# hadleyhzy34/porl

Measured on AMD Instinct MI355X. Metric: gradient-steps/sec (POR update, batch=1024), higher is better.
Workload: dtype f32; 1 GPU; POR S=60 A=2 H=1024 L=2 B=1024/GPU (global 1024), 1000000 -row replay (1000000/GPU) resident in HBM, device sampler + gather + full update per step; parallelism=dp1, global_batch=1024

## Files before the change

### porl_amd/csrc/iql_api.inc

```

namespace {

int64_t add_tensor(std::vector<TensorInfo>& v, int64_t& cur, int rows, int cols) {
  const int64_t off = cur;
  v.push_back({off, rows, cols});
  cur += ru4((int64_t)(rows ? rows : 1) * cols);
  return off;
}

void layout_mlp(MlpLayout& m, std::vector<TensorInfo>& v, int64_t& cur, int in, int hid, int L, int out, bool ln) {
  m.n_lin = L + 1;
  m.ln = ln;
  m.dims[0] = in;
  for (int l = 0; l < L; ++l) m.dims[l + 1] = hid;
  m.dims[L + 1] = out;
  for (int l = 0; l <= L; ++l) {
    m.w[l] = add_tensor(v, cur, m.dims[l + 1], m.dims[l]);
    m.b[l] = add_tensor(v, cur, 0, m.dims[l + 1]);
    if (ln && l < L) {
      m.lnw[l] = add_tensor(v, cur, 0, hid);
      m.lnb[l] = add_tensor(v, cur, 0, hid);
    }
  }
}

struct Workspace {
  int64_t xs_slot[PORL_IQL_SLOTS], xt_slot[PORL_IQL_SLOTS], target_v_slot[PORL_IQL_SLOTS];
  int64_t xn, rew, term;
  int64_t act_v[2][PORL_MAX_HIDDEN], act_t[2][2], act_p[PORL_MAX_HIDDEN];
  int64_t dz_v[2][2], dz_p[2];
  int64_t hp_t[2], hp_v[2];
  int64_t act_q[2][2], hp_q[2];
  int64_t dv[2], dmu;
  int64_t slab_mean, slab_a, slab_b, slab_pa;
  int64_t part_loss, part_min, part_dls;
  int64_t xhat_v[2][PORL_MAX_HIDDEN], rstd_v[2][PORL_MAX_HIDDEN];
  int64_t ln_dg[2], ln_db[2], ln_dh[2];
  int64_t head_part[2], head_loss, head_db[2];
  int64_t pol_w;
  int64_t total;
};

}

struct porl_iql {
  porl_iql_cfg cfg;
  MlpLayout v[2], pol;
  int64_t logstd_off = 0, n_vf = 0, n_pol = 0;
  std::vector<TensorInfo> t_vf, t_pol;
  porl_iql_buffers buf{};
  bool bound = false;
  int device = -1;
  int mode = 0;
  int slot = 0;
  ReduceArgs fin_v{}, fin_p{};
  bool fin_v_pending = false, fin_p_pending = false;
  int batch = 0;
  bool have_pol_target = false;
  bool pol_prefetched = false;
  bool pol_fwd_done = false;
  int pol_nslab = 1;
  int Sp = 0, Dp = 0, Hp = 0, parts_max = 0;
  Workspace ws{};
  Tune tune = g_tune;
};

namespace {

int check_ready(const porl_iql* h, bool need_batch) {
  if (!h) PORL_FAIL(PORL_ERR_INVALID, "null engine");
  if (!h->bound) PORL_FAIL(PORL_ERR_UNBOUND, "porl_iql_bind() has not been called");
  if (need_batch && h->batch <= 0) PORL_FAIL(PORL_ERR_INVALID, "no minibatch loaded (porl_iql_load_batch)");
  return 0;
}
int iql_enter(const porl_iql* h, bool need_batch, const porl_iql_hyper* hp) {
  PORL_TRY(check_ready(h, need_batch));
  if (!hp) PORL_FAIL(PORL_ERR_INVALID, "null hyper-parameters");
  return 0;
// ... 184 lines not shown
  for (int i = 0; i < nnets; ++i) if (!skn_ok4(nets[i].dz, ldz)) return false;
  WgradSkinnyArgs a{};
  a.nnets = nnets; a.B = B; a.H = H; a.S = S; a.ldz = ldz; a.ldx = ldx; a.ldo = S;
  a.tiles_n = cdiv(H, SKN_T);
  skn_split(cdiv(B, SKN_T), h->tune.dw0_slabs, a.nslab, a.rtiles);
  a.slabW_stride = (long)H * S; a.slabC_stride = H;
  for (int i = 0; i < nnets; ++i) {
    a.net[i] = WgradSkinnyNet{nets[i].dz, X, nets[i].sl.W, nets[i].sl.C};
    add_reduce(red, nets[i].gw, nets[i].sl.W, (long)H * S, (long)H * S, a.nslab);
    add_reduce(red, nets[i].gb, nets[i].sl.C, H, H, a.nslab);
  }
  g_phase = phase;
  {
    ProfScope ps("wgrad_skinny_kernel", s, 2.0 * nnets * B * (double)H * S,
                 4.0 * nnets * ((double)B * H + (double)B * S + (double)a.nslab * H * (S + 1)));
    hipLaunchKernelGGL(wgrad_skinny_kernel, dim3(nnets * a.nslab * a.tiles_n), dim3(256), 0, s, a);
  }
  g_phase = "";
  const hipError_t e = hipGetLastError();
  if (e != hipSuccess) { g_err = std::string("wgrad_skinny_kernel: ") + hipGetErrorString(e); *rc = (int)e; }
  return true;
}

int combine_or_defer(ReduceArgs& red, ReduceArgs* defer, hipStream_t s) {
  if (defer) { *defer = red; return 0; }
  return launch_reduce(red, s);
}

int value_forward(porl_iql* h, hipStream_t s, int* parts) {
  const int S = h->cfg.obs_dim, H = h->cfg.hidden_dim, L = h->cfg.n_hidden;
  const Workspace& ws = h->ws;
  for (int l = 0; l < L; ++l) {
    FwdNet nets[4];
    for (int i = 0; i < 2; ++i) {
      nets[i] = twin_fwd_net(h, h->buf.params_tgt, i, l, ws.xn, ws.act_t[i], false, ws.hp_t[i]);
      nets[2 + i] = twin_fwd_net(h, h->buf.params_vf, i, l, ws.xs_slot[h->slot], ws.act_v[i], true, ws.hp_v[i]);
    }
    g_phase = l == 0 ? "V2.L0fwd:" : "V3.fwd:";
    PORL_TRY(fwd_hidden_layer(h, nets, 4, h->batch, l == 0 ? S : H, l == L - 1, parts, false, s));
  }
  g_phase = "V4.head:";
  return PORL_OK;
}

int value_backward_ln(porl_iql* h, const porl_iql_hyper* hp, hipStream_t s, int parts, ReduceArgs* defer) {
  const int B = h->batch, S = h->cfg.obs_dim, H = h->cfg.hidden_dim, L = h->cfg.n_hidden, Hp = h->Hp;
  float* W = h->buf.workspace;
  const Workspace& ws = h->ws;
  const float* Pv = h->buf.params_vf;
  const float* Pt = h->buf.params_tgt;
  float* Gv = h->buf.grads_vf;
  {
    ValueLossArgs a{};
    for (int i = 0; i < 2; ++i) {
      a.hp_t[i] = W + ws.hp_t[i]; a.hp_v[i] = W + ws.hp_v[i];
      a.b_t[i] = Pt + h->v[i].b[L]; a.b_v[i] = Pv + h->v[i].b[L];
      a.dv[i] = W + ws.dv[i];
      a.db_out[i] = Gv + h->v[i].b[L];
    }
    a.rew = W + ws.rew; a.term = W + ws.term; a.target_v = W + ws.target_v_slot[h->slot]; a.stats = h->buf.stats;
    a.B = B; a.parts = parts; a.tau = hp->tau; a.discount = hp->discount; a.inv_batch = hp->inv_batch;
    hipLaunchKernelGGL(value_loss_kernel, dim3(1), dim3(1024), 0, s, a);
    PORL_HIP(hipGetLastError());
  }
  const int nln = cdiv(B, LN_ROWS_PER_BLOCK);
  for (int l = L - 1; l >= 0; --l) {
    const bool top = l == L - 1;
    {
// ... 15 lines not shown
        add_reduce(r, Gv + h->v[i].lnw[l], W + ws.ln_dg[i], H, H, nln);
        add_reduce(r, Gv + h->v[i].lnb[l], W + ws.ln_db[i], H, H, nln);
        if (top) add_reduce(r, Gv + h->v[i].w[L], W + ws.ln_dh[i], H, H, nln);
      }
      PORL_TRY(launch_reduce(r, s));
    }
    ReduceArgs red{};
    GemmGroup g{};
    for (int i = 0; i < 2; ++i) {
      const MlpLayout& m = h->v[i];
      BwdNet n{W + ws.dz_v[i][1], nullptr, Hp, Gv + m.w[l], Gv + m.b[l], Pv + m.w[l], nullptr, nullptr};
      if (l == 0) { n.in = W + ws.xs_slot[h->slot]; n.ldin = h->Sp; }
      else { n.in = W + ws.act_v[i][l - 1]; n.dz_prev = W + ws.dz_v[i][0]; }
      bwd_layer_group(h, g, n, l == 0 ? S : H);
    }
    const int tile = iql_tile(h, g);
    if (l == 0) dw0_splitk(h, g, tile, 2, SLAB_TWIN0, red);
    PORL_TRY(iql_launch(h, g, tile, false, s));
    PORL_TRY(combine_or_defer(red, l == 0 ? defer : nullptr, s));
  }
  return PORL_OK;
}

int value_backward_relu(porl_iql* h, const porl_iql_hyper* hp, hipStream_t s, int parts, ReduceArgs* defer) {
  const int B = h->batch, S = h->cfg.obs_dim, H = h->cfg.hidden_dim, L = h->cfg.n_hidden, Hp = h->Hp;
  float* W = h->buf.workspace;
  const Workspace& ws = h->ws;
  const float* Pv = h->buf.params_vf;
  const float* Pt = h->buf.params_tgt;
  float* Gv = h->buf.grads_vf;
  ReduceArgs red{};
  {
    const int nhb = cdiv(B, HEAD_ROWS_PER_BLOCK);
    HeadBwdArgs a{};
    for (int i = 0; i < 2; ++i) {
      a.Hact[i] = W + ws.act_v[i][L - 1]; a.w[i] = Pv + h->v[i].w[L];
      a.dZ[i] = W + ws.dz_v[i][(L - 1) & 1]; a.part_dw[i] = W + ws.head_part[i];
      a.hp_t[i] = W + ws.hp_t[i]; a.hp_v[i] = W + ws.hp_v[i];
      a.b_t[i] = Pt + h->v[i].b[L]; a.b_v[i] = Pv + h->v[i].b[L];
      a.dv[i] = W + ws.dv[i]; a.part_db[i] = W + ws.head_db[i];
      add_reduce(red, Gv + h->v[i].w[L], W + ws.head_part[i], H, H, nhb);
      add_reduce(red, Gv + h->v[i].b[L], W + ws.head_db[i], 1, 1, nhb);
    }
    a.rew = W + ws.rew; a.term = W + ws.term; a.target_v = W + ws.target_v_slot[h->slot]; a.part_loss = W + ws.head_loss;
    add_reduce(red, h->buf.stats, W + ws.head_loss, 1, 1, nhb, 0, hp->inv_batch);
    a.B = B; a.H = H; a.ld = Hp; a.parts = parts;
    a.tau = hp->tau; a.discount = hp->discount; a.inv_batch = hp->inv_batch;
    ProfScope ps("relu_head_bwd_kernel", s, 0.0, 16.0 * B * H);
    hipLaunchKernelGGL(relu_head_bwd_kernel, dim3(nhb, 2), dim3(256), 0, s, a);
    PORL_HIP(hipGetLastError());
  }
  for (int l = L - 1; l >= 0; --l) {
    if (l == 0) {
      Dw0Net dn[2];
      for (int i = 0; i < 2; ++i) dn[i] = Dw0Net{W + ws.dz_v[i][0], Gv + h->v[i].w[0], Gv + h->v[i].b[0], slabs(h, SlabSet(SLAB_TWIN0 + i))};
      int rc = 0;
      if (dw0_skinny(h, dn, 2, red, "V6.dW0:", s, &rc)) {
        if (rc) return rc;
        break;
      }
    }
    GemmGroup g{};
    for (int i = 0; i < 2; ++i) {
      const MlpLayout& m = h->v[i];
      BwdNet n{W + ws.dz_v[i][l & 1], nullptr, Hp, Gv + m.w[l], Gv + m.b[l], Pv + m.w[l], nullptr, nullptr};
      if (l == 0) { n.in = W + ws.xs_slot[h->slot]; n.ldin = h->Sp; }
      else { n.in = n.mask = W + ws.act_v[i][l - 1]; n.dz_prev = W + ws.dz_v[i][(l - 1) & 1]; }
      bwd_layer_group(h, g, n, l == 0 ? S : H);
    }
    int tile = iql_tile(h, g);
    if (l > 0 && short_blocks(h) && h->tune.vbwd_tile_short >= 0) tile = h->tune.vbwd_tile_short;
    if (l == 0) dw0_splitk(h, g, tile, 2, SLAB_TWIN0, red);
    g_phase = l == 0 ? "V6.dW0:" : "V5.bwd:";
    PORL_TRY(iql_launch(h, g, tile, false, s));
  }
  g_phase = "V7.combine:";
  PORL_TRY(combine_or_defer(red, defer, s));
  g_phase = "";
  return PORL_OK;
}

int value_backward_impl(porl_iql* h, const porl_iql_hyper* hp, hipStream_t s, ReduceArgs* defer) {
  int parts = 0;
  PORL_TRY(value_forward(h, s, &parts));
  return h->cfg.layer_norm ? value_backward_ln(h, hp, s, parts, defer) : value_backward_relu(h, hp, s, parts, defer);
}

int value_adam(porl_iql* h, const porl_iql_hyper* hp, hipStream_t s, const ReduceArgs* fin) {
  g_phase = "V8.";
  const int rc = adam_launch(h->buf.params_vf, h->buf.grads_vf, h->buf.adam_m_vf, h->buf.adam_v_vf, h->buf.params_tgt, h->n_vf,
                             hp->value_lr, hp->value_step, hp->adam_beta1, hp->adam_beta2, hp->adam_eps, hp->ema_beta, s, fin);
  g_phase = "";
  return rc;
}

int policy_adam(porl_iql* h, const porl_iql_hyper* hp, hipStream_t s, const ReduceArgs* fin, const char* phase) {
  g_phase = phase;
  const int rc = adam_launch(h->buf.params_pol, h->buf.grads_pol, h->buf.adam_m_pol, h->buf.adam_v_pol, nullptr, h->n_pol,
                             hp->policy_lr, hp->policy_step, hp->adam_beta1, hp->adam_beta2, hp->adam_eps, 0.0, s, fin);
  g_phase = "";
  return rc;
}

int policy_mean_slabs(porl_iql* h, int B, int* nslab, bool policy, hipStream_t s) {
  const int H = h->cfg.hidden_dim, D = h->cfg.pol_out_dim, L = h->cfg.n_hidden;
  float* W = h->buf.workspace;
  if ((skinny_mask(h) & 2) && D <= SKN_T && H % 4 == 0 && skn_ok4(W + h->ws.act_p[L - 1], h->Hp) &&
      skn_ok4(h->buf.params_pol + h->pol.w[L], H) && h->Dp % 4 == 0) {
    MeanSkinnyArgs a{};
    a.A = W + h->ws.act_p[L - 1]; a.W = h->buf.params_pol + h->pol.w[L]; a.slab = W + h->ws.slab_mean;
    a.B = B; a.H = H; a.D = D; a.lda = h->Hp; a.ldw = H; a.ldo = h->Dp;
    a.tiles_m = cdiv(B, SKN_T);
    skn_split(cdiv(H, SKN_T), a.tiles_m >= 16 ? SK_MAX / 2 : SK_MAX, a.nslab, a.ktiles);
    a.slab_stride = (long)B * h->Dp;
    *nslab = a.nslab;
    ProfScope ps("mean_skinny_kernel", s, 2.0 * B * (double)H * D, 4.0 * ((double)B * H + (double)D * H + (double)a.nslab * B * h->Dp));
    hipLaunchKernelGGL(mean_skinny_kernel, dim3(a.tiles_m * a.nslab), dim3(256), 0, s, a);
    PORL_HIP(hipGetLastError());
    return 0;
  }
  GemmGroup g{};
  g.nprob = 1;
// ... 70 lines not shown
      nets[i] = twin_fwd_net(h, Pt, i, l, ws.xn, ws.act_t[i], false, ws.hp_t[i]);
      nets[2 + i] = twin_fwd_net(h, Pv, i, l, ws.xs_slot[h->slot], ws.act_q[i], false, ws.hp_q[i]);
    }
    nets[4] = policy_fwd_net(h, l, ws.xs_slot[h->slot]);
    g_phase = l == 0 ? "O1.L0fwd:" : "O2.fwd:";
    PORL_TRY(fwd_hidden_layer(h, nets, pre ? 4 : 5, B, l == 0 ? S : H, l == L - 1, &parts, true, s));
  }
  g_phase = "O3.head:";
  PolicyWeightArgs a{};
  for (int i = 0; i < 2; ++i) {
    a.hp_t[i] = W + ws.hp_t[i]; a.hp_v[i] = W + ws.hp_q[i];
    a.b_t[i] = Pt + h->v[i].b[L]; a.b_v[i] = Pv + h->v[i].b[L];
  }
  a.rew = W + ws.rew; a.term = W + ws.term; a.target_v = W + ws.target_v_slot[h->slot]; a.weight = W + ws.pol_w;
  a.B = B; a.parts = parts; a.weight_mode = h->cfg.weight_mode; a.discount = hp->discount; a.alpha = hp->alpha;
  {
    ProfScope ps("policy_weight_kernel", s, 0.0, 4.0 * B * (4.0 * parts + 4.0));
    hipLaunchKernelGGL(policy_weight_kernel, dim3(cdiv(B, PW_ROWS_PER_BLOCK)), dim3(256), 0, s, a);
  }
  PORL_HIP(hipGetLastError());
  return policy_mean_nll(h, hp, s, pre, parts, W + ws.pol_w, "O4.mean:", "O5.");
}

int policy_gradient_half(porl_iql* h, hipStream_t s, ReduceArgs* defer) {
  const int B = h->batch, S = h->cfg.obs_dim, H = h->cfg.hidden_dim, L = h->cfg.n_hidden, D = h->cfg.pol_out_dim;
  const int Hp = h->Hp, Dp = h->Dp;
  float* W = h->buf.workspace;
  const Workspace& ws = h->ws;
  const float* Pp = h->buf.params_pol;
  float* Gp = h->buf.grads_pol;
  const int nblk = cdiv(B, NLL_ROWS_PER_BLOCK);
  h->pol_fwd_done = false;

  ReduceArgs red{};
  add_reduce(red, Gp + h->logstd_off, W + ws.part_dls, D, D, nblk);
  add_reduce(red, h->buf.stats + 1, W + ws.part_loss, 1, 1, nblk);
  add_reduce(red, h->buf.stats + 2, W + ws.part_min, 1, 1, nblk,  1);
  const Slabs out = slabs(h, SLAB_OUT);
  if ((skinny_mask(h) & 4) && D <= SKN_T && H % 4 == 0 && Dp % 4 == 0 && Hp % 4 == 0 && skn_ok4(Pp + h->pol.w[L], H)) {
    OutBwdArgs a{};
    a.dmu = W + ws.dmu; a.W = Pp + h->pol.w[L]; a.A = W + ws.act_p[L - 1];
    a.dZ = W + ws.dz_p[(L - 1) & 1];
    a.slabW = out.W; a.slabC = out.C;
    a.B = B; a.H = H; a.D = D; a.lddmu = Dp; a.ldw = H; a.lda = Hp; a.lddz = Hp;
    a.tiles_n = cdiv(H, SKN_T);
    skn_split(cdiv(B, SKN_T), SK_MAX, a.nslab, a.rtiles);
    a.slabW_stride = out.per; a.slabC_stride = out.perc;
// ... 4 lines not shown
      ProfScope ps("out_bwd_kernel", s, 4.0 * B * (double)H * D, 4.0 * (2.0 * B * H + (double)B * D + (double)D * H + (double)a.nslab * D * H));
      hipLaunchKernelGGL(out_bwd_kernel, dim3(a.nslab * a.tiles_n), dim3(256), 0, s, a);
    }
    g_phase = "";
    PORL_HIP(hipGetLastError());
  } else {
    GemmGroup g{};
    g.nprob = 2;
    g.p[0] = make_prob(GEMM_TN, W + ws.dmu, Dp, W + ws.act_p[L - 1], Hp, Gp + h->pol.w[L], H, D, H, B);
    g.p[0].colsum = Gp + h->pol.b[L];
    g.p[1] = make_prob(GEMM_NN, W + ws.dmu, Dp, Pp + h->pol.w[L], H, W + ws.dz_p[(L - 1) & 1], Hp, B, H, D);
    g.p[1].mask = W + ws.act_p[L - 1]; g.p[1].ldmask = Hp;
    const int tile = D <= 64 ? TILE_64x128 : iql_tile(h, g);
    int bm, bn;
    tile_dims(tile, bm, bn);
    const int sk = pick_splitk(D, H, B, 1, bm, bn);
    if (sk > 1) splitk_to_slabs(g.p[0], out, sk, red);
    g_phase = "P5.outbwd:";
    PORL_TRY(iql_launch(h, g, tile, true, s));
  }
  for (int l = L - 1; l >= 0; --l) {
    if (l == 0) {
      const Dw0Net dn{W + ws.dz_p[0], Gp + h->pol.w[0], Gp + h->pol.b[0], slabs(h, SLAB_POLICY)};
      int rc = 0;
      if (dw0_skinny(h, &dn, 1, red, "P7.dW0:", s, &rc)) {
        if (rc) return rc;
        break;
      }
    }
    GemmGroup g{};
    BwdNet n{W + ws.dz_p[l & 1], nullptr, Hp, Gp + h->pol.w[l], Gp + h->pol.b[l], Pp + h->pol.w[l], nullptr, nullptr};
    if (l == 0) { n.in = W + ws.xs_slot[h->slot]; n.ldin = h->Sp; }
    else { n.in = n.mask = W + ws.act_p[l - 1]; n.dz_prev = W + ws.dz_p[(l - 1) & 1]; }
    bwd_layer_group(h, g, n, l == 0 ? S : H);
    const int tile = iql_tile(h, g);
    if (l == 0) dw0_splitk(h, g, tile, 1, SLAB_POLICY, red);
    g_phase = l == 0 ? "P7.dW0:" : "P6.bwd:";
    PORL_TRY(iql_launch(h, g, tile, true, s));
  }
  g_phase = "P8.combine:";
  PORL_TRY(combine_or_defer(red, defer, s));
  g_phase = "";
  return PORL_OK;
}

int policy_backward_impl(porl_iql* h, const porl_iql_hyper* hp, hipStream_t s, ReduceArgs* defer) {
  PORL_TRY(need_pol_target(h));
  if (!h->pol_fwd_done) PORL_TRY(policy_forward_half(h, hp, s));
  return policy_gradient_half(h, s, defer);
}

int pack_x(porl_iql* h, const float* x, int64_t x_rs, int batch, int64_t dst_off, hipStream_t s) {
  if (!x) PORL_FAIL(PORL_ERR_INVALID, "null input");
  PackArgs a{};
  a.rows = batch; a.njobs = 1;
  a.job[0].src = x; a.job[0].dst = h->buf.workspace + dst_off; a.job[0].src_row_stride = x_rs;
  a.job[0].src_col_stride = 1; a.job[0].cols = h->cfg.obs_dim; a.job[0].ld = h->Sp;
  const long n = (long)batch * h->Sp;
  hipLaunchKernelGGL(pack_kernel, dim3((unsigned)std::min<long>((n + 255) / 256, 1024), 1), dim3(256), 0, s, a);
  PORL_HIP(hipGetLastError());
  return PORL_OK;
}

constexpr size_t SMALL_FWD_LDS_BYTES = 64 * 1024;
bool small_fwd_fits(const porl_iql* h, int batch) {
  return batch >= 1 && batch <= SMALL_FWD_MAX_B &&
         sizeof(float) * (size_t)batch * std::max(h->cfg.obs_dim, h->cfg.hidden_dim) <= SMALL_FWD_LDS_BYTES;
}

// ... 213 lines not shown
  DevGuard _dg(h->device);
  float* W = h->buf.workspace;
  const int slot = next_slot(h);
  IndexedBatchArgs a{};
  a.rows = rows; a.row_stride = (long)row_stride; a.idx = idx;
  a.batch = batch; a.S = state_dim; a.F = F; a.D = D; a.Sp = h->Sp; a.Dp = h->Dp;
  a.target_is_action = target_is_action; a.clamp_target = clamp_target_gt8;
  a.obs_feat = obs_feat; a.obs_rs = (long)obs_rs; a.next_feat = next_feat; a.next_rs = (long)next_rs;
  a.xs = W + h->ws.xs_slot[slot]; a.xn = W + h->ws.xn; a.xt = W + h->ws.xt_slot[slot]; a.rew = W + h->ws.rew; a.term = W + h->ws.term;
  {
    g_phase = "V1.";
    ProfScope ps("indexed_batch_kernel", (hipStream_t)stream, 0.0, 4.0 * batch * (2.0 * h->Sp + h->Dp + 2) * 2.0);
    hipLaunchKernelGGL(indexed_batch_kernel, dim3(cdiv(batch, 4)), dim3(256), 0, (hipStream_t)stream, a);
    g_phase = "";
  }
  PORL_HIP(hipGetLastError());
  iql_batch_loaded(h, batch, true);
  return PORL_OK;
}

int porl_iql_value_backward(porl_iql* h, const porl_iql_hyper* hp, void* stream) {
  PORL_TRY(iql_enter(h, true, hp)); DevGuard _dg(h->device);
  const bool fold = (h->mode & PORL_IQL_MODE_FOLD_COMBINE) != 0;
  h->fin_v = ReduceArgs{};
  PORL_TRY(value_backward_impl(h, hp, (hipStream_t)stream, fold ? &h->fin_v : nullptr));
  h->fin_v_pending = fold;
  return PORL_OK;
}

int porl_iql_value_apply(porl_iql* h, const porl_iql_hyper* hp, void* stream) {
  PORL_TRY(iql_enter(h, false, hp)); DevGuard _dg(h->device);
  const int rc = value_adam(h, hp, (hipStream_t)stream, h->fin_v_pending ? &h->fin_v : nullptr);
  h->fin_v_pending = false;
  return rc;
}

int porl_iql_policy_apply(porl_iql* h, const porl_iql_hyper* hp, void* stream) {
  PORL_TRY(iql_enter(h, false, hp)); DevGuard _dg(h->device);
  const int rc = policy_adam(h, hp, (hipStream_t)stream, h->fin_p_pending ? &h->fin_p : nullptr, "P9.");
  h->fin_p_pending = false;
  return rc;
}

int porl_iql_policy_prefetch(porl_iql* h, void* stream) {
  PORL_TRY(check_ready(h, true));
  PORL_TRY(need_pol_target(h));
  DevGuard _dg(h->device);
  hipStream_t s = (hipStream_t)stream;
  const int S = h->cfg.obs_dim, H = h->cfg.hidden_dim, L = h->cfg.n_hidden;
  int parts = 0;
  for (int l = 0; l < L; ++l) {
    const FwdNet f = policy_fwd_net(h, l, h->ws.xs_slot[h->slot]);
    PORL_TRY(fwd_hidden_layer(h, &f, 1, h->batch, l == 0 ? S : H, l == L - 1, &parts, false, s));
  }
  PORL_TRY(policy_mean_slabs(h, h->batch, &h->pol_nslab, false, s));
  h->pol_prefetched = true;
  return PORL_OK;
}

int porl_iql_policy_forward(porl_iql* h, const porl_iql_hyper* hp, void* stream) {
  PORL_TRY(iql_enter(h, true, hp)); DevGuard _dg(h->device);
  PORL_TRY(need_pol_target(h));
  return h->pol_fwd_done ? PORL_OK : policy_forward_half(h, hp, (hipStream_t)stream);
}

int porl_iql_policy_backward(porl_iql* h, const porl_iql_hyper* hp, void* stream) {
  PORL_TRY(iql_enter(h, true, hp)); DevGuard _dg(h->device);
  const bool fold = (h->mode & PORL_IQL_MODE_FOLD_COMBINE) != 0;
  h->fin_p = ReduceArgs{};
  PORL_TRY(policy_backward_impl(h, hp, (hipStream_t)stream, fold ? &h->fin_p : nullptr));
  h->fin_p_pending = fold;
  return PORL_OK;
}

int porl_iql_step(porl_iql* h, const porl_iql_hyper* hp, void* stream) {
  PORL_TRY(iql_enter(h, true, hp)); DevGuard _dg(h->device);
  hipStream_t s = (hipStream_t)stream;
  ReduceArgs fin{};
  PORL_TRY(value_backward_impl(h, hp, s, h->tune.iql_fold ? &fin : nullptr));
  PORL_TRY(value_adam(h, hp, s, &fin));
  fin = ReduceArgs{};
  PORL_TRY(policy_backward_impl(h, hp, s, h->tune.iql_fold ? &fin : nullptr));
  return policy_adam(h, hp, s, &fin, "P9.");
}

int porl_iql_policy_only_forward(porl_iql* h, const porl_iql_hyper* hp, void* stream) {
  PORL_TRY(iql_enter(h, true, hp)); DevGuard _dg(h->device);
  h->pol_fwd_done = false;
  PORL_TRY(need_pol_target(h));
  return policy_only_forward_half(h, hp, (hipStream_t)stream);
}

int porl_iql_policy_only_step(porl_iql* h, const porl_iql_hyper* hp, void* stream) {
  PORL_TRY(iql_enter(h, true, hp)); DevGuard _dg(h->device);
  PORL_TRY(need_pol_target(h));
  hipStream_t s = (hipStream_t)stream;
  ReduceArgs fin{};
  PORL_TRY(policy_only_forward_half(h, hp, s));
  PORL_TRY(policy_gradient_half(h, s, h->tune.iql_fold ? &fin : nullptr));
  return policy_adam(h, hp, s, &fin, "O9.");
}

int porl_iql_forward_value(porl_iql* h, int which, const float* x, int64_t x_rs, int32_t batch, float* v1_out,
                           float* v2_out, void* stream) {
  PORL_TRY(check_ready(h, false));
  if (!v1_out || !v2_out) PORL_FAIL(PORL_ERR_INVALID, "null output");
  PORL_TRY(check_batch(h, batch));
  DevGuard _dg(h->device);
  hipStream_t s = (hipStream_t)stream;
  const int S = h->cfg.obs_dim, H = h->cfg.hidden_dim, L = h->cfg.n_hidden;
  float* W = h->buf.workspace;
  const Workspace& ws = h->ws;
  const float* P = which ? h->buf.params_tgt : h->buf.params_vf;
  if (small_fwd_fits(h, batch) && !h->cfg.layer_norm && x) {
    const float* in[2] = {x, x};
    long ldin[2] = {(long)x_rs, (long)x_rs};
    for (int l = 0; l <= L; ++l) {
      const float* Wt[2] = {P + h->v[0].w[l], P + h->v[1].w[l]};
      const float* bs[2] = {P + h->v[0].b[l], P + h->v[1].b[l]};
      float* out[2];
// ... 93 lines not shown
```

### porl_amd/csrc/kernels.hpp

```cpp
#pragma once
#include <hip/hip_runtime.h>
#include <stdint.h>

namespace porl {

constexpr float LOG_STD_MIN = -5.0f;
constexpr float LOG_STD_MAX = 2.0f;
constexpr float EXP_ADV_MAX = 100.0f;

__device__ __forceinline__ float wave_sum(float v) {
#pragma unroll
  for (int o = 32; o > 0; o >>= 1) v += __shfl_xor(v, o);
  return v;
}
__device__ __forceinline__ float wave_min(float v) {
#pragma unroll
  for (int o = 32; o > 0; o >>= 1) v = fminf(v, __shfl_xor(v, o));
  return v;
}

struct PackJob {
  const float* src; float* dst;
  long src_row_stride;
  long src_col_stride;
  int cols;
// ... 284 lines not shown
    t *= j.scale;
    if (j.bias) t += j.bias[i % j.ncols];
    if (j.act == 1) t = fmaxf(t, 0.f);
    else if (j.act == 2) t = tanhf(t);
  }
  __syncthreads();
  return t;
}

__global__ __launch_bounds__(256) void multi_reduce_kernel(const ReduceArgs a) {
  __shared__ float sh[REDUCE_LDS_FLOATS];
  const ReduceJob& j = a.job[blockIdx.y];
  const int W = j.width, tx = threadIdx.x % W, ty = threadIdx.x / W;
  for (long i0 = (long)blockIdx.x * W; i0 < j.n; i0 += (long)gridDim.x * W) {
    const float t = reduce_chunk(j, i0, sh);
    if (ty == 0 && i0 + tx < j.n) j.out[i0 + tx] = t;
  }
}

struct AdamScalars { float omb1, beta2, omb2, eps, step_size, bc2_sqrt, ema_beta, omeb; };
constexpr int ADAM_SWEEP_SLABS = 16;
constexpr int MAX_ADAM_REGIONS = 8;
struct AdamRegion { long lo, hi; const float* slab; long stride; int nslab; };
struct AdamArgs {
  float* p; float* g; float* m; float* v; float* tgt;
  long n4;
  long span4;
  int reduce_blocks;
  AdamScalars s;
  int nregions; AdamRegion region[MAX_ADAM_REGIONS];
  int nskip; long skip_lo[MAX_REDUCE_JOBS], skip_hi[MAX_REDUCE_JOBS];
  int job_block0[MAX_REDUCE_JOBS + 1];
  ReduceArgs r;
};

__device__ __forceinline__ float ema1(float t, float p, float omeb, float ema_beta) { return t * omeb + ema_beta * p; }

__device__ __forceinline__ void adam1(float& p, float g, float& m, float& v, const AdamScalars& s) {
  m = m + s.omb1 * (g - m);
  v = v * s.beta2 + s.omb2 * g * g;
  p = p - s.step_size * (m / (sqrtf(v) / s.bc2_sqrt + s.eps));
}

__global__ __launch_bounds__(256) void adam_ema_kernel(const AdamArgs a) {
  __shared__ float sh[REDUCE_LDS_FLOATS];
  const AdamScalars s = a.s;
  if ((int)blockIdx.x < a.reduce_blocks) {
    const int rb = blockIdx.x;
    int ji = 0;
#pragma unroll
    for (int q = 1; q < MAX_REDUCE_JOBS; ++q)
      if (q < a.r.njobs && rb >= a.job_block0[q]) ji = q;
    const ReduceJob& j = a.r.job[ji];
    const long i0 = (long)(rb - a.job_block0[ji]) * j.width;
    const float t = reduce_chunk(j, i0, sh);
    const int tx = threadIdx.x % j.width, ty = threadIdx.x / j.width;
    if (ty == 0 && i0 + tx < j.n) {
      j.out[i0 + tx] = t;
      if (j.adam_off >= 0) {
        const long e = j.adam_off + i0 + tx;
        float pp = a.p[e], mm = a.m[e], vv = a.v[e];
        adam1(pp, t, mm, vv, s);
        a.p[e] = pp; a.m[e] = mm; a.v[e] = vv;
        if (a.tgt) a.tgt[e] = ema1(a.tgt[e], pp, s.omeb, s.ema_beta);
      }
    }
    return;
  }
  float4* p4 = reinterpret_cast<float4*>(a.p);
  float4* g4 = reinterpret_cast<float4*>(a.g);
  float4* m4 = reinterpret_cast<float4*>(a.m);
  float4* v4 = reinterpret_cast<float4*>(a.v);
  float4* t4 = reinterpret_cast<float4*>(a.tgt);
  const long lo4 = (long)(blockIdx.x - a.reduce_blocks) * a.span4, hi4 = min(a.n4, lo4 + a.span4);
  bool special = false;
  for (int q = 0; q < a.nregions; ++q) special = special || (lo4 * 4 < a.region[q].hi && hi4 * 4 > a.region[q].lo);
  for (int q = 0; q < a.nskip; ++q) special = special || (lo4 * 4 < a.skip_hi[q] && hi4 * 4 > a.skip_lo[q]);
  for (long i = lo4 + threadIdx.x; i < hi4; i += 256) {
    float4 gg;
    bool have_g = false;
    if (special) {
      const long e = i * 4;
      bool skip = false;
      for (int q = 0; q < a.nskip; ++q) skip = skip || (e >= a.skip_lo[q] && e < a.skip_hi[q]);
      if (skip) continue;
      for (int q = 0; q < a.nregions; ++q) {
        const AdamRegion& R = a.region[q];
        if (e >= R.lo && e < R.hi) {
          float4 part[8];
#pragma unroll
          for (int u = 0; u < 8; ++u) part[u] = make_float4(0.f, 0.f, 0.f, 0.f);
          const float* base = R.slab + (e - R.lo);
#pragma unroll
          for (int k = 0; k < ADAM_SWEEP_SLABS; ++k)
            if (k < R.nslab) {
              const float4 x = *reinterpret_cast<const float4*>(base + (long)k * R.stride);
              part[k & 7].x += x.x; part[k & 7].y += x.y; part[k & 7].z += x.z; part[k & 7].w += x.w;
// ... 657 lines not shown
```

### porl_amd/csrc/porl_api.hip

```cpp
#include <hip/hip_runtime.h>

#include <algorithm>
#include <cmath>
#include <cstdio>
#include <cstring>
#include <string>
#include <vector>

#include "../../include/porl_hip.h"
#include "gemm_f32.hpp"
#include "gemm_bf16.hpp"
#include "kernels.hpp"
#include "l0_fwd.hpp"
#include "skinny.hpp"
#include "iqn.hpp"
#include "qnet_fused.hpp"
#include "per_tree.hpp"
#include "dist_losses.hpp"
#include "online.hpp"
#include "per_online.hpp"
#include "bcq_mask.hpp"
#include "astar.hpp"
#include "episodes.hpp"
#include "partition.hpp"
// ... 89 lines not shown
  }
};

const float* g_dbg_a_scale = nullptr; const float* g_dbg_a_shift = nullptr; const float* g_dbg_resid = nullptr;
float* g_dbg_cstat = nullptr;
unsigned long long* g_qnet_stamps = nullptr;

constexpr int NUM_CU = 256;
constexpr int SK_MAX = 16;
constexpr int NLL_ROWS_PER_BLOCK = 4;
constexpr int LN_ROWS_PER_BLOCK = 8;
constexpr int HEAD_ROWS_PER_BLOCK = HEAD_ROWS;

struct Tune {
  int tile_map[4] = {TILE_64x128, TILE_64x64, TILE_64x128, TILE_64x64};
  int tile_map_short[4] = {TILE_64x64, TILE_64x64, TILE_64x128, TILE_64x64};
  int vbwd_tile_short = -1;
  int l0_kernel = 1;
  int l0_tile = -1;
  int skinny = 7;
  int skinny_pipelined = -1, skinny_pipelined_max_h = 768;
  int dw0_slabs = 16;
  int iql_fold = 1;
  int gemm_lds_pad = 0, gemm_lds_pad_min_blocks = 0;
  int iql_pad_value = 18432, iql_pad_policy = 0, iql_pad_min_blocks = 4 * NUM_CU, iql_pad_min_k = 0;
  int enc_tile_n96 = 0;
  int enc_gemm_sb = 1;
  int enc_patch_rows = 0;
  int enc_s2d = 0;
  int enc_bf16_operands_only = 0;
  int enc_pconv_mfma = 0;
  int enc_bn_sweep = 0;
  int enc_dense_patch = 0;
  int qnet_fused = 1;
  int qnet_rows16 = 1;
  int qnet_wgrad_share = 11;
  int qnet_two_groups = 1;
} g_tune;

enum TuneClamp { TC_ANY, TC_BOOL, TC_NONNEG, TC_1_16, TC_MASK };
struct TuneKey { const char* key; int Tune::*field; TuneClamp clamp; };
#define TK(key, clamp) {#key, &Tune::key, clamp}
const TuneKey k_tune_keys[] = {
    TK(gemm_lds_pad, TC_NONNEG), TK(gemm_lds_pad_min_blocks, TC_NONNEG), TK(iql_pad_value, TC_NONNEG), TK(iql_pad_policy, TC_NONNEG),
    TK(iql_pad_min_blocks, TC_NONNEG), TK(iql_pad_min_k, TC_NONNEG), TK(qnet_fused, TC_BOOL), TK(qnet_two_groups, TC_BOOL),
    TK(qnet_wgrad_share, TC_1_16), TK(qnet_rows16, TC_BOOL), TK(enc_dense_patch, TC_BOOL), TK(enc_s2d, TC_BOOL), TK(enc_patch_rows, TC_NONNEG),
    TK(enc_gemm_sb, TC_ANY), TK(enc_tile_n96, TC_BOOL), TK(enc_bn_sweep, TC_BOOL), TK(enc_pconv_mfma, TC_BOOL), TK(enc_bf16_operands_only, TC_BOOL),
    TK(iql_fold, TC_BOOL), TK(skinny, TC_MASK), TK(skinny_pipelined, TC_MASK), TK(skinny_pipelined_max_h, TC_ANY), TK(dw0_slabs, TC_1_16),
    TK(l0_tile, TC_ANY), TK(l0_kernel, TC_BOOL), TK(vbwd_tile_short, TC_ANY),
};

int tune_apply(Tune& t, const char* key, int value) {
  if (!key) PORL_FAIL(PORL_ERR_INVALID, "null key");
  for (const TuneKey& k : k_tune_keys) {
    if (strcmp(key, k.key)) continue;
    const TuneClamp c = k.clamp;
    t.*k.field = c == TC_BOOL ? value != 0 : c == TC_NONNEG ? std::max(0, value) : c == TC_1_16 ? std::max(1, std::min(value, 16))
               : c == TC_MASK && value == 1 ? 7 : value;
    return PORL_OK;
  }
  const bool sh = !strncmp(key, "tile_map_short", 14);
  const char* i = key + (sh ? 14 : 8);
  if (!strncmp(key, "tile_map", 8) && *i >= '0' && *i <= '3' && !i[1] && value >= 0 && value < TILE_COUNT) {
    (sh ? t.tile_map_short : t.tile_map)[*i - '0'] = value;
    return PORL_OK;
  }
  PORL_FAIL(PORL_ERR_INVALID, "unknown tuning key '%s'", key);
}

inline int64_t ru4(int64_t x) { return (x + 3) & ~int64_t(3); }
inline int cdiv(int a, int b) { return (a + b - 1) / b; }

// ... 97 lines not shown
  for (int i = 0; i < r.njobs; ++i) maxn = std::max(maxn, r.job[i].n);
  dim3 grid((unsigned)std::min<long>((maxn + 31) / 32, 2048), r.njobs);
  ProfScope ps("multi_reduce_kernel", s, 0.0, 0.0);
  hipLaunchKernelGGL(multi_reduce_kernel, grid, dim3(256), 0, s, r);
  PORL_HIP(hipGetLastError());
  return 0;
}

void add_reduce(ReduceArgs& r, float* out, const float* slab, long n, long stride, int nslab, int op = 0,
                float scale = 1.f) {
  ReduceJob& j = r.job[r.njobs++];
  j.out = out; j.slab = slab; j.bias = nullptr; j.n = n; j.stride = stride; j.nslab = nslab; j.ncols = 1; j.act = 0;
  j.op = op; j.scale = scale; j.adam_off = -1;
  j.width = nslab > 64 ? 4 : 32;
}

int feistel_half_bits(int64_t n_rows) {
  int bits = 1;
  while ((int64_t(1) << bits) < n_rows) ++bits;
  return std::max(1, (bits + 1) / 2);
}

int adam_launch(float* p, float* g, float* m, float* v, float* tgt, int64_t n, double lr, int step,
                       double b1, double b2, double eps, double ema_beta, hipStream_t s, const ReduceArgs* fin = nullptr) {
  if (n < 0 || n % 4) PORL_FAIL(PORL_ERR_INVALID, "adam range must be a non-negative multiple of 4 floats");
  if (step < 1) PORL_FAIL(PORL_ERR_INVALID, "adam step must be >= 1");
  if (n == 0 && !(fin && fin->njobs)) return PORL_OK;
  AdamArgs a{};
  a.p = p; a.g = g; a.m = m; a.v = v; a.tgt = tgt;
  const double bc1 = 1.0 - std::pow(b1, (double)step);
  const double bc2 = 1.0 - std::pow(b2, (double)step);
  a.s.step_size = (float)(lr / bc1);
  a.s.bc2_sqrt = (float)std::sqrt(bc2);
  a.s.omb1 = (float)(1.0 - b1); a.s.beta2 = (float)b2; a.s.omb2 = (float)(1.0 - b2);
  a.s.eps = (float)eps; a.s.ema_beta = (float)ema_beta; a.s.omeb = (float)(1.0 - ema_beta);
  a.n4 = n / 4;
  const int sweep_blocks = (int)std::min<long>((a.n4 + 255) / 256, 1 << 20);
  a.span4 = sweep_blocks ? ((a.n4 + sweep_blocks - 1) / sweep_blocks + 255) / 256 * 256 : 256;
  int reduce_blocks = 0;
  double extra_bytes = 0.0;
  if (fin) {
    for (int q = 0; q < fin->njobs; ++q) {
      ReduceJob j = fin->job[q];
      const bool inside = j.out >= g && j.out + j.n <= g + n;
      const long off = inside ? (long)(j.out - g) : -1;
      extra_bytes += 4.0 * (double)j.n * j.nslab;
      const bool plain = j.op == 0 && j.scale == 1.f && !j.bias && j.act == 0;
      if (inside && plain && j.nslab <= ADAM_SWEEP_SLABS && off % 4 == 0 && j.n % 4 == 0 && j.stride % 4 == 0 &&
          aligned16(j.slab) && a.nregions < MAX_ADAM_REGIONS) {
        AdamRegion& R = a.region[a.nregions++];
        R.lo = off; R.hi = off + j.n; R.slab = j.slab; R.stride = j.stride; R.nslab = j.nslab;
        continue;
      }
      if (inside) {
        if (off % 4) PORL_FAIL(PORL_ERR_INVALID, "gradient tensors start on 16-byte boundaries");
        j.adam_off = off;
        a.skip_lo[a.nskip] = off; a.skip_hi[a.nskip] = ru4(off + j.n); ++a.nskip;
      } else {
        j.adam_off = -1;
      }
      a.job_block0[a.r.njobs] = reduce_blocks;
      a.r.job[a.r.njobs++] = j;
      reduce_blocks += (int)((j.n + j.width - 1) / j.width);
    }
    a.job_block0[a.r.njobs] = reduce_blocks;
  }
  ProfScope ps("adam_ema_kernel", s, 0.0, (double)n * (tgt ? 36.0 : 28.0) + extra_bytes);
  a.reduce_blocks = reduce_blocks;
  hipLaunchKernelGGL(adam_ema_kernel, dim3(sweep_blocks + reduce_blocks), dim3(256), 0, s, a);
  PORL_HIP(hipGetLastError());
  return PORL_OK;
}

}

extern "C" {

int porl_abi_version(void) { return PORL_ABI_VERSION; }
const char* porl_last_error(void) { return g_err.c_str(); }

int porl_gemm_f32(int mode, int tile, int32_t M, int32_t N, int32_t K, const float* A, int32_t lda, const float* B,
                  int32_t ldb, float* C, int32_t ldc, const float* bias, int act, const float* mask, int32_t ldmask,
                  int splitk, float* slab, void* stream) {
  if (mode < 0 || mode > 2) PORL_FAIL(PORL_ERR_INVALID, "mode must be 0..2");
  if (M < 1 || N < 1 || K < 0 || !A || !B || !C) PORL_FAIL(PORL_ERR_INVALID, "bad GEMM arguments");
  if (splitk > 1 && !slab) PORL_FAIL(PORL_ERR_INVALID, "splitk > 1 needs a slab buffer");
  if (splitk > 1 && ldc != N) PORL_FAIL(PORL_ERR_INVALID, "splitk > 1 needs a dense C (ldc == N)");
  DevGuard _dg(device_of(C));
  hipStream_t s = (hipStream_t)stream;
  GemmGroup g{};
  g.nprob = 1;
  g.p[0] = make_prob(mode, A, lda, B, ldb, C, ldc, M, N, K);
// ... 412 lines not shown
```

Baseline: 3058 gradient-steps/sec.

## Fuse input-layer weight-gradient GEMM into the Adam/EMA kernel

Instead of launching a separate skinny weight-gradient kernel for the first layer and reducing its split-K slabs inside Adam, the Adam kernel now gets extra blocks. Each block computes a 32x32 tile of dz^T·x with MFMA over the whole batch and applies the Adam and EMA update directly to those elements. The bias gradient is computed in the same blocks. This is meant to remove a kernel launch, the slab writes and the slab re-reads. In exchange, each new block walks the full batch serially and the grid has relatively few such tiles, which can lengthen the kernel's critical path.

```diff
diff --git a/porl_amd/csrc/iql_api.inc b/porl_amd/csrc/iql_api.inc
--- a/porl_amd/csrc/iql_api.inc
+++ b/porl_amd/csrc/iql_api.inc
@@ -41,6 +41,8 @@
   int64_t total;
 };
 
+struct AdamFin { ReduceArgs red; AdamDw0 dw0; };
+
 }
 
 struct porl_iql {
@@ -53,7 +55,7 @@
   int device = -1;
   int mode = 0;
   int slot = 0;
-  ReduceArgs fin_v{}, fin_p{};
+  AdamFin fin_v{}, fin_p{};
   bool fin_v_pending = false, fin_p_pending = false;
   int batch = 0;
   bool have_pol_target = false;
@@ -284,8 +286,22 @@
   return true;
 }
 
-int combine_or_defer(ReduceArgs& red, ReduceArgs* defer, hipStream_t s) {
-  if (defer) { *defer = red; return 0; }
+bool dw0_in_adam(const porl_iql* h, const Dw0Net* nets, int nnets, const float* G, AdamFin* defer) {
+  const int B = h->batch, H = h->cfg.hidden_dim, S = h->cfg.obs_dim, ldx = h->Sp, ldz = h->Hp;
+  const Tune& t = h->tune;
+  if (!defer || !t.dw0_in_adam || (t.dw0_in_adam < 0 && (int64_t)B * H < t.dw0_in_adam_min_bh)) return false;
+  const float* X = h->buf.workspace + h->ws.xs_slot[h->slot];
+  if (S > 64 || S % 4 || H % 4 || nnets > ADW_MAX_NETS || !skn_ok4(X, ldx) || ldz % 4) return false;
+  for (int i = 0; i < nnets; ++i) if (!skn_ok4(nets[i].dz, ldz)) return false;
+  AdamDw0& d = defer->dw0;
+  d = AdamDw0{};
+  d.nnets = nnets; d.B = B; d.H = H; d.S = S; d.ldz = ldz; d.ldx = ldx;
+  for (int i = 0; i < nnets; ++i) d.net[i] = AdamDw0Net{nets[i].dz, X, (long)(nets[i].gw - G), (long)(nets[i].gb - G)};
+  return true;
+}
+
+int combine_or_defer(ReduceArgs& red, AdamFin* defer, hipStream_t s) {
+  if (defer) { defer->red = red; return 0; }
   return launch_reduce(red, s);
 }
 
@@ -305,7 +321,7 @@
   return PORL_OK;
 }
 
-int value_backward_ln(porl_iql* h, const porl_iql_hyper* hp, hipStream_t s, int parts, ReduceArgs* defer) {
+int value_backward_ln(porl_iql* h, const porl_iql_hyper* hp, hipStream_t s, int parts, AdamFin* defer) {
   const int B = h->batch, S = h->cfg.obs_dim, H = h->cfg.hidden_dim, L = h->cfg.n_hidden, Hp = h->Hp;
   float* W = h->buf.workspace;
   const Workspace& ws = h->ws;
@@ -367,7 +383,7 @@
   return PORL_OK;
 }
 
-int value_backward_relu(porl_iql* h, const porl_iql_hyper* hp, hipStream_t s, int parts, ReduceArgs* defer) {
+int value_backward_relu(porl_iql* h, const porl_iql_hyper* hp, hipStream_t s, int parts, AdamFin* defer) {
   const int B = h->batch, S = h->cfg.obs_dim, H = h->cfg.hidden_dim, L = h->cfg.n_hidden, Hp = h->Hp;
   float* W = h->buf.workspace;
   const Workspace& ws = h->ws;
@@ -399,6 +415,7 @@
     if (l == 0) {
       Dw0Net dn[2];
       for (int i = 0; i < 2; ++i) dn[i] = Dw0Net{W + ws.dz_v[i][0], Gv + h->v[i].w[0], Gv + h->v[i].b[0], slabs(h, SlabSet(SLAB_TWIN0 + i))};
+      if (dw0_in_adam(h, dn, 2, Gv, defer)) break;
       int rc = 0;
       if (dw0_skinny(h, dn, 2, red, "V6.dW0:", s, &rc)) {
         if (rc) return rc;
@@ -425,24 +442,26 @@
   return PORL_OK;
 }
 
-int value_backward_impl(porl_iql* h, const porl_iql_hyper* hp, hipStream_t s, ReduceArgs* defer) {
+int value_backward_impl(porl_iql* h, const porl_iql_hyper* hp, hipStream_t s, AdamFin* defer) {
   int parts = 0;
   PORL_TRY(value_forward(h, s, &parts));
   return h->cfg.layer_norm ? value_backward_ln(h, hp, s, parts, defer) : value_backward_relu(h, hp, s, parts, defer);
 }
 
-int value_adam(porl_iql* h, const porl_iql_hyper* hp, hipStream_t s, const ReduceArgs* fin) {
+int value_adam(porl_iql* h, const porl_iql_hyper* hp, hipStream_t s, const AdamFin* fin) {
   g_phase = "V8.";
   const int rc = adam_launch(h->buf.params_vf, h->buf.grads_vf, h->buf.adam_m_vf, h->buf.adam_v_vf, h->buf.params_tgt, h->n_vf,
-                             hp->value_lr, hp->value_step, hp->adam_beta1, hp->adam_beta2, hp->adam_eps, hp->ema_beta, s, fin);
+                             hp->value_lr, hp->value_step, hp->adam_beta1, hp->adam_beta2, hp->adam_eps, hp->ema_beta, s,
+                             fin ? &fin->red : nullptr, fin ? &fin->dw0 : nullptr);
   g_phase = "";
   return rc;
 }
 
-int policy_adam(porl_iql* h, const porl_iql_hyper* hp, hipStream_t s, const ReduceArgs* fin, const char* phase) {
+int policy_adam(porl_iql* h, const porl_iql_hyper* hp, hipStream_t s, const AdamFin* fin, const char* phase) {
   g_phase = phase;
   const int rc = adam_launch(h->buf.params_pol, h->buf.grads_pol, h->buf.adam_m_pol, h->buf.adam_v_pol, nullptr, h->n_pol,
-                             hp->policy_lr, hp->policy_step, hp->adam_beta1, hp->adam_beta2, hp->adam_eps, 0.0, s, fin);
+                             hp->policy_lr, hp->policy_step, hp->adam_beta1, hp->adam_beta2, hp->adam_eps, 0.0, s,
+                             fin ? &fin->red : nullptr, fin ? &fin->dw0 : nullptr);
   g_phase = "";
   return rc;
 }
@@ -559,7 +578,7 @@
   return policy_mean_nll(h, hp, s, pre, parts, W + ws.pol_w, "O4.mean:", "O5.");
 }
 
-int policy_gradient_half(porl_iql* h, hipStream_t s, ReduceArgs* defer) {
+int policy_gradient_half(porl_iql* h, hipStream_t s, AdamFin* defer) {
   const int B = h->batch, S = h->cfg.obs_dim, H = h->cfg.hidden_dim, L = h->cfg.n_hidden, D = h->cfg.pol_out_dim;
   const int Hp = h->Hp, Dp = h->Dp;
   float* W = h->buf.workspace;
@@ -610,6 +629,7 @@
   for (int l = L - 1; l >= 0; --l) {
     if (l == 0) {
       const Dw0Net dn{W + ws.dz_p[0], Gp + h->pol.w[0], Gp + h->pol.b[0], slabs(h, SLAB_POLICY)};
+      if (dw0_in_adam(h, &dn, 1, Gp, defer)) break;
       int rc = 0;
       if (dw0_skinny(h, &dn, 1, red, "P7.dW0:", s, &rc)) {
         if (rc) return rc;
@@ -632,7 +652,7 @@
   return PORL_OK;
 }
 
-int policy_backward_impl(porl_iql* h, const porl_iql_hyper* hp, hipStream_t s, ReduceArgs* defer) {
+int policy_backward_impl(porl_iql* h, const porl_iql_hyper* hp, hipStream_t s, AdamFin* defer) {
   PORL_TRY(need_pol_target(h));
   if (!h->pol_fwd_done) PORL_TRY(policy_forward_half(h, hp, s));
   return policy_gradient_half(h, s, defer);
@@ -892,7 +912,7 @@
 int porl_iql_value_backward(porl_iql* h, const porl_iql_hyper* hp, void* stream) {
   PORL_TRY(iql_enter(h, true, hp)); DevGuard _dg(h->device);
   const bool fold = (h->mode & PORL_IQL_MODE_FOLD_COMBINE) != 0;
-  h->fin_v = ReduceArgs{};
+  h->fin_v = AdamFin{};
   PORL_TRY(value_backward_impl(h, hp, (hipStream_t)stream, fold ? &h->fin_v : nullptr));
   h->fin_v_pending = fold;
   return PORL_OK;
@@ -937,7 +957,7 @@
 int porl_iql_policy_backward(porl_iql* h, const porl_iql_hyper* hp, void* stream) {
   PORL_TRY(iql_enter(h, true, hp)); DevGuard _dg(h->device);
   const bool fold = (h->mode & PORL_IQL_MODE_FOLD_COMBINE) != 0;
-  h->fin_p = ReduceArgs{};
+  h->fin_p = AdamFin{};
   PORL_TRY(policy_backward_impl(h, hp, (hipStream_t)stream, fold ? &h->fin_p : nullptr));
   h->fin_p_pending = fold;
   return PORL_OK;
@@ -946,10 +966,10 @@
 int porl_iql_step(porl_iql* h, const porl_iql_hyper* hp, void* stream) {
   PORL_TRY(iql_enter(h, true, hp)); DevGuard _dg(h->device);
   hipStream_t s = (hipStream_t)stream;
-  ReduceArgs fin{};
+  AdamFin fin{};
   PORL_TRY(value_backward_impl(h, hp, s, h->tune.iql_fold ? &fin : nullptr));
   PORL_TRY(value_adam(h, hp, s, &fin));
-  fin = ReduceArgs{};
+  fin = AdamFin{};
   PORL_TRY(policy_backward_impl(h, hp, s, h->tune.iql_fold ? &fin : nullptr));
   return policy_adam(h, hp, s, &fin, "P9.");
 }
@@ -965,7 +985,7 @@
   PORL_TRY(iql_enter(h, true, hp)); DevGuard _dg(h->device);
   PORL_TRY(need_pol_target(h));
   hipStream_t s = (hipStream_t)stream;
-  ReduceArgs fin{};
+  AdamFin fin{};
   PORL_TRY(policy_only_forward_half(h, hp, s));
   PORL_TRY(policy_gradient_half(h, s, h->tune.iql_fold ? &fin : nullptr));
   return policy_adam(h, hp, s, &fin, "O9.");
diff --git a/porl_amd/csrc/kernels.hpp b/porl_amd/csrc/kernels.hpp
--- a/porl_amd/csrc/kernels.hpp
+++ b/porl_amd/csrc/kernels.hpp
@@ -1,6 +1,7 @@
 #pragma once
 #include <hip/hip_runtime.h>
 #include <stdint.h>
+#include "gemm_f32.hpp"
 
 namespace porl {
 
@@ -331,16 +332,35 @@
 constexpr int ADAM_SWEEP_SLABS = 16;
 constexpr int MAX_ADAM_REGIONS = 8;
 struct AdamRegion { long lo, hi; const float* slab; long stride; int nslab; };
+constexpr int ADW_MAX_NETS = 2;
+constexpr int ADW_T = 32;
+constexpr int ADW_KC = 16;
+constexpr int ADW_LD = ADW_T + 4;
+constexpr int ADW_DEPTH = 6;
+constexpr int ADW_STAGE = 2 * ADW_KC * ADW_LD;
+constexpr int ADW_COMB_LD = ADW_T + 1;
+struct AdamDw0Net { const float* dz; const float* x; long w_off, b_off; };
+struct AdamDw0 {
+  int nnets, B, H, S;
+  int ldz, ldx;
+  int tiles_h, tiles_s;
+  AdamDw0Net net[ADW_MAX_NETS];
+};
+constexpr int ADAM_LDS_FLOATS = 4 * ADW_T * ADW_COMB_LD + 8 * ADW_T;
+static_assert(ADAM_LDS_FLOATS >= 2 * ADW_STAGE && ADAM_LDS_FLOATS >= 64 * 5 && ADW_DEPTH % 2 == 0, "adam_ema_kernel LDS");
+
 struct AdamArgs {
   float* p; float* g; float* m; float* v; float* tgt;
   long n4;
   long span4;
+  int dw0_blocks;
   int reduce_blocks;
   AdamScalars s;
   int nregions; AdamRegion region[MAX_ADAM_REGIONS];
-  int nskip; long skip_lo[MAX_REDUCE_JOBS], skip_hi[MAX_REDUCE_JOBS];
+  int nskip; long skip_lo[MAX_REDUCE_JOBS + ADW_MAX_NETS], skip_hi[MAX_REDUCE_JOBS + ADW_MAX_NETS];
   int job_block0[MAX_REDUCE_JOBS + 1];
   ReduceArgs r;
+  AdamDw0 dw0;
 };
 
 __device__ __forceinline__ float ema1(float t, float p, float omeb, float ema_beta) { return t * omeb + ema_beta * p; }
@@ -351,11 +371,111 @@
   p = p - s.step_size * (m / (sqrtf(v) / s.bc2_sqrt + s.eps));
 }
 
-__global__ __launch_bounds__(256) void adam_ema_kernel(const AdamArgs a) {
-  __shared__ float sh[REDUCE_LDS_FLOATS];
+__device__ __forceinline__ void adam_finish1(const AdamArgs& a, long e, float t) {
+  a.g[e] = t;
+  float pp = a.p[e], mm = a.m[e], vv = a.v[e];
+  adam1(pp, t, mm, vv, a.s);
+  a.p[e] = pp; a.m[e] = mm; a.v[e] = vv;
+  if (a.tgt) a.tgt[e] = ema1(a.tgt[e], pp, a.s.omeb, a.s.ema_beta);
+}
+
+__device__ __forceinline__ float4 adw_load(const float* src, long ld, int B, int b0, int r) {
+  return *reinterpret_cast<const float4*>(src + (long)min(b0 + r, B - 1) * ld);
+}
+__device__ __forceinline__ float4 adw_keep(const float4 v, bool ok) {
+  return make_float4(ok ? v.x : 0.f, ok ? v.y : 0.f, ok ? v.z : 0.f, ok ? v.w : 0.f);
+}
+
+__device__ __forceinline__ void adam_dw0_block(const AdamArgs& a, int pb, float* lds) {
+  const AdamDw0& d = a.dw0;
+  const int t = threadIdx.x, lane = t & 63, wave = t >> 6, li = lane & 31, kh = lane >> 5;
+  const int per_net = d.tiles_h * d.tiles_s;
+  const int ni = pb / per_net, rem = pb - ni * per_net;
+  const int th = rem / d.tiles_s, ts = rem - th * d.tiles_s;
+  const AdamDw0Net& n = d.net[ni];
+  const int h0 = th * ADW_T, s0 = ts * ADW_T;
+  const int nch = (d.B + ADW_KC - 1) / ADW_KC;
+  const bool isx = t >= 128;
+  const int prow = (t & 127) >> 3, pc4 = (t & 7) * 4;
+  const bool cin = isx ? s0 + pc4 < d.S : h0 + pc4 < d.H;
+  const float* src = (isx ? n.x : n.dz) + (cin ? (isx ? s0 : h0) + pc4 : 0);
+  const long ld = isx ? d.ldx : d.ldz;
+  float* park = lds + (isx ? ADW_KC * ADW_LD : 0) + prow * ADW_LD + pc4;
+  float4 ring[ADW_DEPTH];
+#pragma unroll
+  for (int u = 0; u < ADW_DEPTH; ++u) {
+    ring[u] = adw_load(src, ld, d.B, u * ADW_KC, prow);
+    __builtin_amdgcn_sched_barrier(0);
+  }
+  f32x16 acc;
+#pragma unroll
+  for (int r = 0; r < 16; ++r) acc[r] = 0.f;
+  float cs = 0.f;
+  const int col = t & 31, rg = t >> 5;
+  for (int c = 0; c < nch; c += ADW_DEPTH) {
+#pragma unroll
+    for (int u = 0; u < ADW_DEPTH; ++u) {
+      const int ch = c + u;
+      *reinterpret_cast<float4*>(park + (u & 1) * ADW_STAGE) = adw_keep(ring[u], cin && ch * ADW_KC + prow < d.B);
+      ring[u] = adw_load(src, ld, d.B, (ch + ADW_DEPTH) * ADW_KC, prow);
+      __syncthreads();
+      const float* Zl = lds + (u & 1) * ADW_STAGE;
+      const float* zp = Zl + (4 * wave + kh) * ADW_LD + li;
+      const float* xp = zp + ADW_KC * ADW_LD;
+      acc = __builtin_amdgcn_mfma_f32_32x32x2f32(zp[0], xp[0], acc, 0, 0, 0);
+      acc = __builtin_amdgcn_mfma_f32_32x32x2f32(zp[2 * ADW_LD], xp[2 * ADW_LD], acc, 0, 0, 0);
+      cs = (cs + Zl[2 * rg * ADW_LD + col]) + Zl[(2 * rg + 1) * ADW_LD + col];
+    }
+  }
+  __syncthreads();
+  float* comb = lds;
+  float* csum = lds + 4 * ADW_T * ADW_COMB_LD;
+#pragma unroll
+  for (int r = 0; r < 16; ++r)
+    comb[(wave * ADW_T + (r & 3) + 8 * (r >> 2) + 4 * kh) * ADW_COMB_LD + li] = acc[r];
+  csum[rg * ADW_T + col] = cs;
+  __syncthreads();
+#pragma unroll
+  for (int q0 = 0; q0 < 4; q0 += 2) {
+    float w[2], pp[2], mm[2], vv[2], tt[2];
+    long e[2];
+    bool ok[2];
+#pragma unroll
+    for (int q = 0; q < 2; ++q) {
+      const int row = rg + 8 * (q0 + q), h = h0 + row, sc = s0 + col;
+      const float* c0 = comb + row * ADW_COMB_LD + col;
+      w[q] = ((c0[0] + c0[ADW_T * ADW_COMB_LD]) + c0[2 * ADW_T * ADW_COMB_LD]) + c0[3 * ADW_T * ADW_COMB_LD];
+      ok[q] = h < d.H && sc < d.S;
+      e[q] = ok[q] ? n.w_off + (long)h * d.S + sc : n.w_off;
+      pp[q] = a.p[e[q]]; mm[q] = a.m[e[q]]; vv[q] = a.v[e[q]];
+      tt[q] = a.tgt ? a.tgt[e[q]] : 0.f;
+    }
+#pragma unroll
+    for (int q = 0; q < 2; ++q) {
+      adam1(pp[q], w[q], mm[q], vv[q], a.s);
+      if (ok[q]) {
+        a.g[e[q]] = w[q]; a.p[e[q]] = pp[q]; a.m[e[q]] = mm[q]; a.v[e[q]] = vv[q];
+        if (a.tgt) a.tgt[e[q]] = ema1(tt[q], pp[q], a.s.omeb, a.s.ema_beta);
+      }
+    }
+  }
+  if (ts == 0 && t < ADW_T && h0 + t < d.H) {
+    float b = csum[t];
+#pragma unroll
+    for (int q = 1; q < 8; ++q) b += csum[q * ADW_T + t];
+    adam_finish1(a, n.b_off + h0 + t, b);
+  }
+}
+
+__global__ __launch_bounds__(256, 8) void adam_ema_kernel(const AdamArgs a) {
+  __shared__ __attribute__((aligned(16))) float sh[ADAM_LDS_FLOATS];
   const AdamScalars s = a.s;
-  if ((int)blockIdx.x < a.reduce_blocks) {
-    const int rb = blockIdx.x;
+  if ((int)blockIdx.x < a.dw0_blocks) {
+    adam_dw0_block(a, blockIdx.x, sh);
+    return;
+  }
+  if ((int)blockIdx.x < a.dw0_blocks + a.reduce_blocks) {
+    const int rb = blockIdx.x - a.dw0_blocks;
     int ji = 0;
 #pragma unroll
     for (int q = 1; q < MAX_REDUCE_JOBS; ++q)
@@ -381,7 +501,7 @@
   float4* m4 = reinterpret_cast<float4*>(a.m);
   float4* v4 = reinterpret_cast<float4*>(a.v);
   float4* t4 = reinterpret_cast<float4*>(a.tgt);
-  const long lo4 = (long)(blockIdx.x - a.reduce_blocks) * a.span4, hi4 = min(a.n4, lo4 + a.span4);
+  const long lo4 = (long)(blockIdx.x - a.dw0_blocks - a.reduce_blocks) * a.span4, hi4 = min(a.n4, lo4 + a.span4);
   bool special = false;
   for (int q = 0; q < a.nregions; ++q) special = special || (lo4 * 4 < a.region[q].hi && hi4 * 4 > a.region[q].lo);
   for (int q = 0; q < a.nskip; ++q) special = special || (lo4 * 4 < a.skip_hi[q] && hi4 * 4 > a.skip_lo[q]);
diff --git a/porl_amd/csrc/porl_api.hip b/porl_amd/csrc/porl_api.hip
--- a/porl_amd/csrc/porl_api.hip
+++ b/porl_amd/csrc/porl_api.hip
@@ -135,6 +135,7 @@
   int skinny_pipelined = -1, skinny_pipelined_max_h = 768;
   int dw0_slabs = 16;
   int iql_fold = 1;
+  int dw0_in_adam = -1, dw0_in_adam_min_bh = 1 << 18;
   int gemm_lds_pad = 0, gemm_lds_pad_min_blocks = 0;
   int iql_pad_value = 18432, iql_pad_policy = 0, iql_pad_min_blocks = 4 * NUM_CU, iql_pad_min_k = 0;
   int enc_tile_n96 = 0;
@@ -160,7 +161,7 @@
     TK(qnet_wgrad_share, TC_1_16), TK(qnet_rows16, TC_BOOL), TK(enc_dense_patch, TC_BOOL), TK(enc_s2d, TC_BOOL), TK(enc_patch_rows, TC_NONNEG),
     TK(enc_gemm_sb, TC_ANY), TK(enc_tile_n96, TC_BOOL), TK(enc_bn_sweep, TC_BOOL), TK(enc_pconv_mfma, TC_BOOL), TK(enc_bf16_operands_only, TC_BOOL),
     TK(iql_fold, TC_BOOL), TK(skinny, TC_MASK), TK(skinny_pipelined, TC_MASK), TK(skinny_pipelined_max_h, TC_ANY), TK(dw0_slabs, TC_1_16),
-    TK(l0_tile, TC_ANY), TK(l0_kernel, TC_BOOL), TK(vbwd_tile_short, TC_ANY),
+    TK(l0_tile, TC_ANY), TK(l0_kernel, TC_BOOL), TK(vbwd_tile_short, TC_ANY), TK(dw0_in_adam, TC_ANY), TK(dw0_in_adam_min_bh, TC_NONNEG),
 };
 
 int tune_apply(Tune& t, const char* key, int value) {
@@ -304,7 +305,8 @@
 }
 
 int adam_launch(float* p, float* g, float* m, float* v, float* tgt, int64_t n, double lr, int step,
-                       double b1, double b2, double eps, double ema_beta, hipStream_t s, const ReduceArgs* fin = nullptr) {
+                       double b1, double b2, double eps, double ema_beta, hipStream_t s, const ReduceArgs* fin = nullptr,
+                       const AdamDw0* dw0 = nullptr) {
   if (n < 0 || n % 4) PORL_FAIL(PORL_ERR_INVALID, "adam range must be a non-negative multiple of 4 floats");
   if (step < 1) PORL_FAIL(PORL_ERR_INVALID, "adam step must be >= 1");
   if (n == 0 && !(fin && fin->njobs)) return PORL_OK;
@@ -347,9 +349,29 @@
     }
     a.job_block0[a.r.njobs] = reduce_blocks;
   }
-  ProfScope ps("adam_ema_kernel", s, 0.0, (double)n * (tgt ? 36.0 : 28.0) + extra_bytes);
+  double flops = 0.0;
+  if (dw0 && dw0->nnets) {
+    const AdamDw0& d = *dw0;
+    if (d.nnets > ADW_MAX_NETS || d.B < 1 || d.H < 1 || d.S < 1 || d.S > 64 || d.H % 4 || d.S % 4 || d.ldz % 4 || d.ldx % 4 ||
+        d.ldz < d.H || d.ldx < d.S)
+      PORL_FAIL(PORL_ERR_INVALID, "input-layer product inside Adam: shapes do not qualify");
+    a.dw0 = d;
+    a.dw0.tiles_h = cdiv(d.H, ADW_T); a.dw0.tiles_s = cdiv(d.S, ADW_T);
+    for (int i = 0; i < d.nnets; ++i) {
+      const AdamDw0Net& w = d.net[i];
+      if (!aligned16(w.dz) || !aligned16(w.x) || w.w_off < 0 || w.b_off < 0 || w.w_off % 4 || w.b_off % 4 ||
+          w.w_off + (long)d.H * d.S > n || w.b_off + d.H > n)
+        PORL_FAIL(PORL_ERR_INVALID, "input-layer product inside Adam: operands do not qualify");
+      a.skip_lo[a.nskip] = w.w_off; a.skip_hi[a.nskip] = ru4(w.w_off + (long)d.H * d.S); ++a.nskip;
+      a.skip_lo[a.nskip] = w.b_off; a.skip_hi[a.nskip] = ru4(w.b_off + d.H); ++a.nskip;
+    }
+    a.dw0_blocks = d.nnets * a.dw0.tiles_h * a.dw0.tiles_s;
+    flops = 2.0 * d.nnets * d.B * (double)d.H * d.S;
+    extra_bytes += 4.0 * ((double)d.nnets * d.B * d.H + (double)d.B * d.S);
+  }
+  ProfScope ps("adam_ema_kernel", s, flops, (double)n * (tgt ? 36.0 : 28.0) + extra_bytes);
   a.reduce_blocks = reduce_blocks;
-  hipLaunchKernelGGL(adam_ema_kernel, dim3(sweep_blocks + reduce_blocks), dim3(256), 0, s, a);
+  hipLaunchKernelGGL(adam_ema_kernel, dim3(a.dw0_blocks + reduce_blocks + sweep_blocks), dim3(256), 0, s, a);
   PORL_HIP(hipGetLastError());
   return PORL_OK;
 }
```

After: 3031 gradient-steps/sec. No clear change (-0.9%).
